# yixuan/spectra

Measured on AMD Instinct MI355X. Metric: eigenpairs_per_sec, higher is better.
Workload: dtype f64

## Files before the change

### include/mispec.h

```cpp
#ifndef MISPEC_H
#define MISPEC_H

#include <stdint.h>

#ifdef __cplusplus
extern "C" {
#endif

#define MISPEC_OK 0
#define MISPEC_EINVAL (-1)
#define MISPEC_ELOGIC (-2)
#define MISPEC_ERUNTIME (-3)

typedef struct mispec_ctx mispec_ctx;
typedef struct mispec_csr mispec_csr;
typedef struct mispec_fac mispec_fac;

const char* mispec_last_error(void);
const char* mispec_version(void);

int mispec_set_option(const char* name, const char* value);
const char* mispec_get_option(const char* name);

int mispec_ctx_create(int device, void* hip_stream, mispec_ctx** out);
// ... 25 lines not shown
int mispec_csr_from_csc(mispec_ctx* ctx, int64_t n_rows, int64_t n_cols, const int32_t* colptr_host,
                        const int32_t* rowind_host, const double* val_host, mispec_csr** out);
int mispec_csr_from_triangle(mispec_ctx* ctx, int64_t n, const int32_t* outer_host, const int32_t* inner_host,
                             const double* val_host, char uplo, int row_major, mispec_csr** out);
int mispec_csr_synth_band(mispec_ctx* ctx, int64_t n, uint64_t seed, const int64_t* offsets, int noff, int symmetric,
                          mispec_csr** out);
int mispec_csr_destroy(mispec_csr* A);
int64_t mispec_csr_rows(const mispec_csr* A);
int64_t mispec_csr_cols(const mispec_csr* A);
int64_t mispec_csr_local_rows(const mispec_csr* A);
int64_t mispec_csr_local_nnz(const mispec_csr* A);
int mispec_csr_offset_codes(const mispec_csr* A);
int mispec_csr_use_offset_codes(mispec_csr* A, int enable);
int mispec_csr_use_windows(mispec_csr* A, int enable);
int mispec_csr_windows_info(const mispec_csr* A, int64_t* blocks, int64_t* covered_entries, int64_t* lds_doubles);
int mispec_csr_windows_in_use(const mispec_csr* A);
int mispec_csr_windows_table(const mispec_csr* A, int32_t* records_out, int64_t capacity);
int mispec_csr_windows_host(int64_t n_rows, int64_t n_cols, int64_t row_begin, const int32_t* rowptr, const int32_t* colind,
                            int32_t* records_out);
int mispec_csr_spmv_format(const mispec_csr* A);
int mispec_csr_set_spmv_format(mispec_csr* A, int format);
double mispec_csr_spmv_bytes(const mispec_csr* A, int stored);
int mispec_csr_dia_info(const mispec_csr* A, int* ndia, int* nstored, int* nmirrored, int* lead_blocks);
int mispec_dia_sym_plan(const int32_t* offsets, int nd, int64_t reach, int32_t* out_flags, int* lead_blocks);
int mispec_csr_coeff(const mispec_csr* A, int64_t i, int64_t j, double* out);
int mispec_csr_download(const mispec_csr* A, int32_t* rowptr_host, int32_t* colind_host, double* val_host);

int mispec_spmv(const mispec_csr* A, const double* x_dev, double* y_dev);
int mispec_spmv_host(const mispec_csr* A, const double* x_host, double* y_host);
int mispec_spmm_host(const mispec_csr* A, const double* X_host, int64_t ldx, int k, double* Y_host, int64_t ldy);
int mispec_spmm(const mispec_csr* A, const double* X_dev, int64_t ldx, int k, double* Y_dev, int64_t ldy);
int mispec_spmm_plan(int k, int forced_panel, int* widths_out, int cap, int* count);
int mispec_csr_reorder(mispec_csr* A, int method, int* applied);
int mispec_csr_reordering(const mispec_csr* A, double* far_before, double* far_after);
int mispec_csr_permutation(const mispec_csr* A, int32_t* perm_out);
int mispec_csr_tiles_info(const mispec_csr* A, int64_t* segments, int64_t* entries, int64_t* padding, int64_t* chunks);
int mispec_csr_staged_info(const mispec_csr* A, int64_t* bins, int64_t* slots, int64_t* batches, int64_t* chunks);
int mispec_last_ingest_info(double* seconds_out, int count);
int mispec_ingest_threads(void);
int mispec_mirror_triangle_host(int64_t n, const int32_t* outer, const int32_t* inner, const double* val, char uplo, int row_major,
                                int32_t* rowptr_out, int32_t* colind_out, double* val_out, int64_t capacity, int64_t* nnz_out);
int mispec_tiles_spmv_host(int64_t nrows, int64_t ncols, const int32_t* rowptr, const int32_t* colind, const double* val,
                           const double* x, double* y, int* built, int64_t* stats);
int mispec_staged_spmv_host(int64_t nrows, int64_t ncols, const int32_t* rowptr, const int32_t* colind, const double* val,
                            const double* x, double* y, int* built, int64_t* stats);
int mispec_rcm_order(int64_t n, const int32_t* rowptr, const int32_t* colind, int symmetric_pattern, int32_t* perm_out,
// ... 177 lines not shown
```

### spectra_amd/__init__.py

```python
import ctypes as C
import enum
import os

import numpy as np

from . import _capi
from ._capi import MispecError, Profile, build_library, check, lib

__all__ = ["SortRule", "CompInfo", "Context", "SparseSymMatProd", "SparseGenMatProd", "SparseSymShiftSolve", "SymEigsSolver",
           "SymEigsShiftSolver", "GenEigsSolver", "SVDMatOp", "PartialSVDSolver", "SparseRegularInverse", "SparseCholesky", "SymGEigsSolver", "SymShiftInvert", "SymGEigsShiftSolver", "SparseGenRealShiftSolve", "GenEigsRealShiftSolver", "shard_block",
           "Factorization", "tridiag_qr", "tridiag_eigen", "hess_qr", "double_shift_qr", "hess_schur", "hess_eigen", "MispecError", "build_library", "shard_range", "BAND_OFFSETS", "SYNTH_SEED",
           "SparseHermMatProd", "DenseHermMatProd", "HermEigsSolver", "spmm_plan", "dia_sym_plan"]

BAND_OFFSETS = (1, 2, 3, 1000, 1001, 100000, 100001)
SYNTH_SEED = 20240607


ORTH_MODES = {"reference": 0, "onesweep": 1, "onesweep-eager": 1 | 0x100, "onesweep-recorrect": 1 | 0x200, "onesweep-restart-check": 1 | 0x400,
              "onesweep-onered": 1 | 0x800, "onesweep-twored": 1 | 0x1000, "onesweep-onered-eager": 1 | 0x800 | 0x100}


def _orth_mode_value(mode):
    if isinstance(mode, str):
        if mode not in ORTH_MODES:
# ... 252 lines not shown
        return ms.value

    def algorithmic_bytes(self):
        return 12.0 * self.nnz() + 4.0 * (self.local_rows() + 1) + 8.0 * self.cols() + 8.0 * self.local_rows()

    def offset_codes(self):
        return int(lib().mispec_csr_offset_codes(self.h))

    def use_offset_codes(self, enable=True):
        check(lib().mispec_csr_use_offset_codes(self.h, 1 if enable else 0))

    def use_windows(self, enable=True):
        check(lib().mispec_csr_use_windows(self.h, -1 if enable is None else (1 if enable else 0)))

    def windows_info(self):
        a, b, c = C.c_int64(0), C.c_int64(0), C.c_int64(0)
        check(lib().mispec_csr_windows_info(self.h, C.byref(a), C.byref(b), C.byref(c)))
        return {"blocks": a.value, "covered_entries": b.value, "lds_doubles": c.value}

    def dia_info(self):
        a, b, c, d = C.c_int(0), C.c_int(0), C.c_int(0), C.c_int(0)
        check(lib().mispec_csr_dia_info(self.h, C.byref(a), C.byref(b), C.byref(c), C.byref(d)))
        return {"ndia": a.value, "nstored": b.value, "nmirrored": c.value, "lead_blocks": d.value}

    def windows_in_use(self):
        return bool(lib().mispec_csr_windows_in_use(self.h))

    def windows_table(self):
        nb = (self.local_rows() + 255) // 256
        out = np.empty((nb, 32), dtype=np.int32)
        check(lib().mispec_csr_windows_table(self.h, _ip(out), out.size))
        return out

    def spmv_format(self):
        return int(lib().mispec_csr_spmv_format(self.h))

    def set_spmv_format(self, fmt=-1):
        check(lib().mispec_csr_set_spmv_format(self.h, int(fmt)))

    def stored_bytes(self):
        return float(lib().mispec_csr_spmv_bytes(self.h, 1))

    def staged_info(self):
        a, b, c, d = C.c_int64(0), C.c_int64(0), C.c_int64(0), C.c_int64(0)
        check(lib().mispec_csr_staged_info(self.h, C.byref(a), C.byref(b), C.byref(c), C.byref(d)))
        return {"bins": a.value, "slots": b.value, "batches": c.value, "chunks": d.value}
# ... 1393 lines not shown
```

### spectra_amd/_capi.py

```python
import ctypes as C
import os
import subprocess

_PKG = os.path.dirname(os.path.abspath(__file__))
LIB_PATH = os.path.join(_PKG, "libmispec.so")
EXTRAS_LIB_PATH = os.path.join(_PKG, "libmispec_extras.so")
EXTRAS_PREFIXES = ("mispec_davidson_", "mispec_zdense_", "mispec_zfac_", "mispec_zcsr_", "mispec_hermeigs_")
CSRC = os.path.join(_PKG, "csrc")

MISPEC_OK, MISPEC_EINVAL, MISPEC_ELOGIC, MISPEC_ERUNTIME = 0, -1, -2, -3


class MispecError(RuntimeError):
    """HIP / RCCL failure or a failed small decomposition (std::runtime_error in the C++ API)."""


def build_library(force=False, verbose=False):
    cmd = ["make", "-C", CSRC, "-j8"] + (["-B"] if force else [])
    out = subprocess.run(cmd, stdout=subprocess.PIPE, stderr=subprocess.STDOUT, text=True)
    if verbose or out.returncode != 0:
        print(out.stdout)
    if out.returncode != 0:
        raise RuntimeError("building libmispec.so failed")
    return LIB_PATH
# ... 44 lines not shown
    "mispec_loopback_destroy": (C.c_int, [_vp]),
    "mispec_shard_block": (C.c_int64, [C.c_int64, C.c_int]),
    "mispec_shard_range": (C.c_int, [C.c_int64, C.c_int, C.c_int, _lp, _lp]),
    "mispec_csr_upload": (C.c_int, [_vp, C.c_int64, C.c_int64, _ip, _ip, _dp, _vpp]),
    "mispec_csr_from_csc": (C.c_int, [_vp, C.c_int64, C.c_int64, _ip, _ip, _dp, _vpp]),
    "mispec_csr_from_triangle": (C.c_int, [_vp, C.c_int64, _ip, _ip, _dp, C.c_char, C.c_int, _vpp]),
    "mispec_csr_synth_band": (C.c_int, [_vp, C.c_int64, C.c_uint64, _lp, C.c_int, C.c_int, _vpp]),
    "mispec_csr_destroy": (C.c_int, [_vp]),
    "mispec_csr_rows": (C.c_int64, [_vp]),
    "mispec_csr_cols": (C.c_int64, [_vp]),
    "mispec_csr_local_rows": (C.c_int64, [_vp]),
    "mispec_csr_local_nnz": (C.c_int64, [_vp]),
    "mispec_csr_offset_codes": (C.c_int, [_vp]),
    "mispec_csr_use_offset_codes": (C.c_int, [_vp, C.c_int]),
    "mispec_csr_use_windows": (C.c_int, [_vp, C.c_int]),
    "mispec_csr_windows_info": (C.c_int, [_vp, _lp, _lp, _lp]),
    "mispec_csr_windows_table": (C.c_int, [_vp, _ip, C.c_int64]),
    "mispec_csr_windows_in_use": (C.c_int, [_vp]),
    "mispec_csr_windows_host": (C.c_int, [C.c_int64, C.c_int64, C.c_int64, _ip, _ip, _ip]),
    "mispec_csr_spmv_format": (C.c_int, [_vp]),
    "mispec_csr_set_spmv_format": (C.c_int, [_vp, C.c_int]),
    "mispec_csr_spmv_bytes": (C.c_double, [_vp, C.c_int]),
    "mispec_csr_dia_info": (C.c_int, [_vp, C.POINTER(C.c_int), C.POINTER(C.c_int), C.POINTER(C.c_int), C.POINTER(C.c_int)]),
    "mispec_dia_sym_plan": (C.c_int, [_ip, C.c_int, C.c_int64, _ip, C.POINTER(C.c_int)]),
    "mispec_csr_coeff": (C.c_int, [_vp, C.c_int64, C.c_int64, _dp]),
    "mispec_csr_download": (C.c_int, [_vp, _ip, _ip, _dp]),
    "mispec_spmv": (C.c_int, [_vp, _vp, _vp]),
    "mispec_spmv_host": (C.c_int, [_vp, _dp, _dp]),
    "mispec_spmm_host": (C.c_int, [_vp, _dp, C.c_int64, C.c_int, _dp, C.c_int64]),
    "mispec_spmv_time": (C.c_int, [_vp, _vp, _vp, C.c_int, C.POINTER(C.c_float)]),
    "mispec_spmm": (C.c_int, [_vp, _vp, C.c_int64, C.c_int, _vp, C.c_int64]),
    "mispec_spmm_time": (C.c_int, [_vp, _vp, C.c_int64, C.c_int, _vp, C.c_int64, C.c_int, C.POINTER(C.c_float)]),
    "mispec_spmm_plan": (C.c_int, [C.c_int, C.c_int, C.POINTER(C.c_int), C.c_int, C.POINTER(C.c_int)]),
    "mispec_symshift_level_plan": (C.c_int, [C.c_int64, C.c_int64, C.c_int, _lp, _lp, _lp, _lp]),
    "mispec_symshift_create": (C.c_int, [_vp, C.c_int64, _ip, _ip, _dp, C.c_char, C.c_int, _vpp]),
    "mispec_symshift_destroy": (C.c_int, [_vp]),
    "mispec_symshift_rows": (C.c_int64, [_vp]),
    "mispec_symshift_bandwidth": (C.c_int, [_vp, _lp, _lp, C.POINTER(C.c_int)]),
    "mispec_csr_tiles_info": (C.c_int, [_vp, _lp, _lp, _lp, _lp]),
    "mispec_csr_staged_info": (C.c_int, [_vp, _lp, _lp, _lp, _lp]),
    "mispec_csr_reorder": (C.c_int, [_vp, C.c_int, C.POINTER(C.c_int)]),
    "mispec_csr_reordering": (C.c_int, [_vp, _dp, _dp]),
    "mispec_csr_permutation": (C.c_int, [_vp, _ip]),
    "mispec_staged_spmv_host": (C.c_int, [C.c_int64, C.c_int64, _ip, _ip, _dp, _dp, _dp, C.POINTER(C.c_int), C.POINTER(C.c_int64)]),
    "mispec_tiles_spmv_host": (C.c_int, [C.c_int64, C.c_int64, _ip, _ip, _dp, _dp, _dp, C.POINTER(C.c_int), C.POINTER(C.c_int64)]),
    "mispec_rcm_order": (C.c_int, [C.c_int64, _ip, _ip, C.c_int, _ip, C.POINTER(C.c_int), C.POINTER(C.c_int64)]),
# ... 218 lines not shown
```

### spectra_amd/csrc/common.hpp

```cpp
#pragma once

#include <hip/hip_runtime.h>

#include <cstdint>
#include <cstdio>
#include <cstdlib>
#include <new>
#include <functional>
#include <utility>
#include <stdexcept>
#include <string>
#include <vector>

#include "../../include/mispec.h"
#include "../../include/mispec_extras.h"

namespace mispec {

struct Error : std::runtime_error
{
    int code;
    Error(int c, const std::string& m) : std::runtime_error(m), code(c) {}
};

// ... 88 lines not shown
    PinnedBuf() {}
    PinnedBuf(const PinnedBuf&) = delete;
    PinnedBuf& operator=(const PinnedBuf&) = delete;
    ~PinnedBuf()
    {
        if (p)
            (void) hipHostFree(p);
    }
    void alloc(size_t count)
    {
        if (p)
            (void) hipHostFree(p);
        p = nullptr;
        MISPEC_HIP(hipHostMalloc(reinterpret_cast<void**>(&p), count * sizeof(T), hipHostMallocDefault));
        n = count;
    }
};

inline int64_t round_up(int64_t x, int64_t m) { return (x + m - 1) / m * m; }

enum class Opt
{
    orth, one_reduction, orth_kernel, host_turn, small, restart_sync, host_steps, overlap, csr_win, spec_corr, exchange, reorder,
    spmv_staged, spmv_tiles, spmm, dia_sym, host_threads, shift, count
};
enum class Orth { onesweep, onesweep_eager, reference };
enum class OrthKernel { dma, dma2, reg, unset };
enum class HostTurn { fast, copy };
enum class Small { host, host_serial, device };
enum class Exchange { allgather, halo, unset };
enum class Reorder { automatic, rcm, none };
enum class Tri { automatic, off, on };
enum class DiaSym { automatic, off, all };
enum class Spmm { automatic, off, w2, w4, w8 };
int option_choice(Opt o);
template <typename E>
E option_choice(Opt o, E unset)
{
    const int i = option_choice(o);
    return i < 0 ? unset : E(i);
}
bool option_flag(Opt o, bool unset);
int option_int(Opt o, int unset);
struct ShiftOptions
{
    int lds = 1;
    int batch = 0;
    int lanes = 0;
    int block_inverse = 256;
    int factor_host = 0;
    int wave = 1;
    int profile = 0;
};
ShiftOptions shift_options();

void* big_host_alloc(size_t bytes);
// ... 57 lines not shown
```

### spectra_amd/csrc/csr_dia.hip

```cpp
#include "csr_kernels.hpp"

#include <algorithm>
#include <cstdlib>
#include <cstring>
#include <numeric>
#include <vector>

using namespace mispec;

namespace {

constexpr int kMaxDia = 32;
constexpr int kDiaGroup = 8;
constexpr int64_t kDiaSymReach = 131072;
constexpr bool kMirrorNontemporal = false;
constexpr int kDiaMir = 8;

__global__ __launch_bounds__(256) void k_build_dia(const int32_t* __restrict__ rowptr, const uint8_t* __restrict__ codes,
                                                   const double* __restrict__ val, const int32_t* __restrict__ pos_of_code,
                                                   int64_t nloc, int64_t ld, double* __restrict__ dia, int* __restrict__ bad, int nd_blocked)
{
    const int64_t r = int64_t(blockIdx.x) * 256 + threadIdx.x;
    if (r >= nloc)
        return;
// ... 490 lines not shown
        __syncthreads();
        const int wv = tid >> 6, lane = tid & 63;
#pragma unroll
        for (int h = 0; h < 2; h++)
        {
            const int k = 2 * wv + h;
            const double s = wave_reduce_sum(cbuf[64 * k + lane]);
            if (lane == 0)
                red[k] = s;
        }
        __syncthreads();
        if (tid == 0)
            epi.partials[lb] = (red[0] + red[1]) + (red[2] + red[3]);
    }
    else
    {
        if (have1)
            *reinterpret_cast<double2*>(y + row0 + r0) = make_double2(acc0, acc1);
        else if (have0)
            y[row0 + r0] = acc0;
    }
}

int dia_sym_rule(const int32_t* offs, int nd, int64_t reach, int32_t* flags)
{
    int64_t kmax = 0;
    for (int i = 0; i < nd; i++)
    {
        flags[i] = 0;
        const int64_t k = -int64_t(offs[i]);
        if (k <= 0 || (reach >= 0 && k > reach))
            continue;
        for (int j = 0; j < nd; j++)
            if (int64_t(offs[j]) == k)
                flags[i] = 1;
        if (flags[i])
            kmax = std::max(kmax, k);
    }
    return int((kmax + 255) / 256);
}

mispec_dia_plan make_plan(const int32_t* offs, int nd, const int32_t* mirrored)
{
    mispec_dia_plan pl;
    int64_t kmax = 0;
    for (int i = 0; i < nd; i++)
// ... 1 lines not shown
        pl.shift[i] = mirrored[i] ? -offs[i] : 0;
        if (!mirrored[i])
            pl.src[i] = pl.nstored++ + mispec_dia_plan::kStream;
        else
            kmax = std::max<int64_t>(kmax, -int64_t(offs[i]));
    }
    pl.lead = int((kmax + 255) / 256);
    for (int i = 0; i < nd; i++)
        if (mirrored[i])
            for (int j = 0; j < nd; j++)
                if (offs[j] == -offs[i])
                {
                    pl.src[j] = pl.slot(j);
                    pl.src[i] = pl.slot(j) + (kMirrorNontemporal ? mispec_dia_plan::kStream : 0);
                }
    for (int i = nd; i < 32; i++)
    {
        pl.src[i] = pl.src[nd - 1];
        pl.shift[i] = pl.shift[nd - 1];
    }
    return pl;
}

}

extern "C" int mispec_dia_sym_plan(const int32_t* offsets, int nd, int64_t reach, int32_t* out_flags, int* lead_blocks)
{
    return guarded([&] {
        MISPEC_REQUIRE(nd >= 0 && nd <= kMaxDia && (nd == 0 || (offsets && out_flags)), "mispec_dia_sym_plan: bad argument");
        const int lead = dia_sym_rule(offsets, nd, reach, out_flags);
        if (lead_blocks)
            *lead_blocks = lead;
    });
}

extern "C" int mispec_csr_dia_info(const mispec_csr* A, int* ndia, int* nstored, int* nmirrored, int* lead_blocks)
{
    return guarded([&] {
        MISPEC_REQUIRE(A, "mispec_csr_dia_info: NULL argument");
        if (ndia)
            *ndia = A->ndia;
        if (nstored)
            *nstored = A->ndia ? A->dia_plan.nstored : 0;
        if (nmirrored)
            *nmirrored = A->ndia ? A->ndia - A->dia_plan.nstored : 0;
        if (lead_blocks)
            *lead_blocks = A->ndia ? A->dia_plan.lead : 0;
    });
}

namespace mispec {

void build_dia(mispec_csr& A, const std::vector<int32_t>& dict)
{
    const int64_t nloc = A.local_rows();
    const int nd = int(dict.size());
    if (nd == 0 || nd > kMaxDia || nloc == 0 || double(A.nnz) < 0.75 * double(nd) * double(nloc))
        return;
    std::vector<int32_t> order(static_cast<size_t>(nd)), pos(static_cast<size_t>(nd)), offs(static_cast<size_t>(nd));
    std::iota(order.begin(), order.end(), 0);
    std::sort(order.begin(), order.end(), [&](int32_t a, int32_t b) { return dict[size_t(a)] < dict[size_t(b)]; });
    for (int k = 0; k < nd; k++)
    {
        pos[size_t(order[size_t(k)])] = k;
        offs[size_t(k)] = dict[size_t(order[size_t(k)])];
    }
    constexpr bool blocked = true;
    const int64_t ld = round_up(nloc, 256);
    DevBuf<int32_t> d_pos;
    DevBuf<int> d_bad;
// ... 87 lines not shown
    hipLaunchKernelGGL(k_dia_compact, dim3(nblk), dim3(256), 0, st, A.dia.p, nd, nloc, plan, packed.p);
    MISPEC_HIP(hipGetLastError());
    MISPEC_HIP(hipStreamSynchronize(st));
    A.dia.swap(packed);
    A.dia_plan = plan;
}

void launch_spmv_dia(const mispec_csr& A, const SpmvLaunch& L)
{
    const dim3 grid = L.grid, block = L.block;
    const int64_t nloc = L.nloc;
    const int nblocks = L.nblocks;
    const SpmvEpilogue* epi = L.epi;
    const SpmvEpilogue e = L.e;
    const hipEvent_t ev_start = L.ev_start, ev_stop = L.ev_stop;
    const double* x_dev = L.x_dev;
    double* y_dev = L.y_dev;
        const DiaArgs da{A.dia.p, A.dia_off.p, A.dia_ld, A.ndia, int(A.n_cols - 1), A.row_begin, A.dia_plan};
        const bool mir = A.dia_plan.nstored != A.ndia;
        MISPEC_REQUIRE(!mir || (A.dia_ld == 0 && A.dia_win.nc > 0), "diagonal storage: a mirror plan needs the block layout and x windows");
        const bool dia2 = A.dia_win.nc > 0 && A.dia_ld == 0 && A.ndia <= 2 * kDiaGroup &&
                          (reinterpret_cast<uintptr_t>(y_dev) & 15) == 0 &&
                          (!epi || ((reinterpret_cast<uintptr_t>(e.v_rows) & 15) == 0 && (reinterpret_cast<uintptr_t>(e.v_prev) & 15) == 0));
        if (dia2)
        {
            const size_t lds2 = size_t(A.dia_win.total + 256) * sizeof(double);
            const dim3 block2(128);
            const int ng = (A.ndia + kDiaGroup - 1) / kDiaGroup;
            const bool post = epi && e.post_scale_state;
#define MISPEC_DIA2_LAUNCH(E, G, W, P)                                                                                                  \
    do                                                                                                                                  \
    {                                                                                                                                   \
        if (ev_start && ev_stop)                                                                                                        \
            hipExtLaunchKernelGGL((k_spmv_dia_win2<E, G, W, P>), grid, block2, lds2, A.ctx->stream, ev_start, ev_stop, 0, da, A.dia_win, \
                                  x_dev, y_dev, nloc, nblocks, e);                                                                      \
        else                                                                                                                            \
            hipLaunchKernelGGL((k_spmv_dia_win2<E, G, W, P>), grid, block2, lds2, A.ctx->stream, da, A.dia_win, x_dev, y_dev, nloc,     \
                               nblocks, e);                                                                                             \
    } while (0)
#define MISPEC_DIA2_W(E, G, P)               \
    do                                       \
    {                                        \
        if (A.dia_win.nc <= 4)               \
            MISPEC_DIA2_LAUNCH(E, G, 4, P);  \
        else if (A.dia_win.nc <= 6)          \
            MISPEC_DIA2_LAUNCH(E, G, 6, P);  \
// ... 138 lines not shown
```

### spectra_amd/csrc/ctx.hip

```cpp
#include "common.hpp"

#include <dlfcn.h>
#include <rccl/rccl.h>

#include <algorithm>
#include <condition_variable>
#include <exception>
#include <thread>
#include <cstring>
#include <mutex>

namespace mispec {
static thread_local std::string g_last_error;
void set_last_error(const std::string& msg) { g_last_error = msg; }

void* big_host_alloc(size_t bytes)
{
    void* q = std::malloc(bytes ? bytes : 1);
    if (!q)
        throw std::bad_alloc();
    return q;
}

namespace {
// ... 18 lines not shown
    {Opt::orth_kernel, "orth_kernel", "MISPEC_ORTH_KERNEL", Kind::choice, {"dma", "dma2", "reg"}, 0, 0,
     "orthogonalisation passes through an LDS-DMA ring of three / two slots or through registers (unset: dma from 131072 rows)"},
    {Opt::host_turn, "host_turn", "MISPEC_HOST_TURN", Kind::choice, {"fast", "copy"}, 0, 0,
     "restart's host turn: pinned-memory kernels or hipMemcpy"},
    {Opt::small, "small", "MISPEC_SMALL", Kind::choice, {"host", "host-serial", "device"}, 0, 0,
     "where the ncv x ncv work of a restart runs"},
    {Opt::restart_sync, "restart_sync", "MISPEC_RESTART_SYNC", Kind::choice, {"0", "1"}, 0, 0, "synchronising fused restart"},
    {Opt::host_steps, "host_steps", "MISPEC_HOST_STEPS", Kind::choice, {"0", "1"}, 0, 0, "host-synchronous steps"},
    {Opt::overlap, "overlap", "MISPEC_OVERLAP", Kind::choice, {"0", "1"}, 0, 0,
     "sharded product: overlap of the exchange with the local rows (default 1)"},
    {Opt::csr_win, "csr_win", "MISPEC_CSR_WIN", Kind::choice, {"0", "1"}, 0, 0, "x windows of the int32 CSR kernel (default 1)"},
    {Opt::spec_corr, "spec_corr", "MISPEC_SPEC_CORR", Kind::integer, {}, 1, 4,
     "corrections enqueued speculatively per step (unset: 2, 1 when sharded)"},
    {Opt::exchange, "exchange", "MISPEC_EXCHANGE", Kind::choice, {"allgather", "halo"}, 0, 0,
     "sharded product: the all-gather or the neighbour exchange (unset: the exchange when the halos are small)"},
    {Opt::reorder, "reorder", "MISPEC_REORDER", Kind::choice, {"auto", "rcm", "none"}, 0, 0,
     "reverse Cuthill-McKee ordering at ingest and of the shift solve"},
    {Opt::spmv_staged, "spmv_staged", "MISPEC_SPMV_STAGED", Kind::choice, {"auto", "0", "1"}, 0, 0, "staged SpMV format"},
    {Opt::spmv_tiles, "spmv_tiles", "MISPEC_SPMV_TILES", Kind::choice, {"auto", "0", "1"}, 0, 0, "column-blocked tile SpMV format"},
    {Opt::spmm, "spmm", "MISPEC_SPMM", Kind::choice, {"auto", "0", "2", "4", "8"}, 0, 0,
     "widest panel of a block product (0: one SpMV per column)"},
    {Opt::dia_sym, "dia_sym", "MISPEC_DIA_SYM", Kind::choice, {"auto", "0", "all"}, 0, 0,
     "diagonal storage: lower diagonals read from their mirrored upper partner (auto: those within reach, 0: none, all)"},
    {Opt::host_threads, "host_threads", "MISPEC_HOST_THREADS", Kind::integer, {}, 1, kMaxInt,
     "upper bound on the host threads of the ingest and of the shift solve's host-side factorisation"},
    {Opt::shift, "shift", "MISPEC_SHIFT", Kind::shift, {}, 0, 0, "kernel variants of the banded shift solve"},
};
static_assert(sizeof(kOptions) / sizeof(kOptions[0]) == size_t(Opt::count), "one entry per option");
constexpr bool entries_in_order()
{
    for (size_t i = 0; i < size_t(Opt::count); i++)
        if (kOptions[i].id != Opt(i))
            return false;
    return true;
}
static_assert(entries_in_order(), "kOptions is indexed by Opt");

struct ShiftKey
{
    const char* key;
    const char* values[kMaxValues];
    int ShiftOptions::*field;
};
const ShiftKey kShiftKeys[] = {
    {"lds", {"0", "1"}, &ShiftOptions::lds},
    {"batch", {"8", "16", "32"}, &ShiftOptions::batch},
// ... 609 lines not shown
```

### spectra_amd/csrc/orth_dma.hip

```cpp
#include "krylov.hpp"

using namespace mispec;

namespace {

constexpr int kThreads = 256;
constexpr int kNW = 4;
constexpr int kRows = 128;
typedef __attribute__((address_space(3))) char lds_char;

__device__ __forceinline__ double wave_sum(double v)
{
#pragma unroll
    for (int off = 32; off > 0; off >>= 1)
        v += __shfl_down(v, off, 64);
    return v;
}
__device__ __forceinline__ double wave_max(double v)
{
#pragma unroll
    for (int off = 32; off > 0; off >>= 1)
        v = fmax(v, __shfl_down(v, off, 64));
    return v;
}

template <bool NT>
__device__ __forceinline__ void dma16(const double* gsrc, unsigned lds_dst)
{
    unsigned keep;
    if (NT)
        asm volatile("s_mov_b32 %0, m0\n\ts_mov_b32 m0, %2\n\ts_nop 0\n\tglobal_load_lds_dwordx4 %1, off nt\n\ts_mov_b32 m0, %0"
                     : "=&s"(keep)
                     : "v"(gsrc), "s"(lds_dst)
                     : "memory");
    else
        asm volatile("s_mov_b32 %0, m0\n\ts_mov_b32 m0, %2\n\ts_nop 0\n\tglobal_load_lds_dwordx4 %1, off\n\ts_mov_b32 m0, %0"
                     : "=&s"(keep)
                     : "v"(gsrc), "s"(lds_dst)
                     : "memory");
}

template <int MAXS, int DEPTH, bool ONERED>
__global__ __launch_bounds__(kThreads, 1) void k_orth_lagged_dma(OrthArgs a)
{
    constexpr int NL = MAXS + 1;
    constexpr int kRegion = kRows;
    constexpr int kSlotDoubles = kNW * NL * kRegion;
    extern __shared__ __attribute__((aligned(16))) char smem[];
    double* ring = reinterpret_cast<double*>(smem);
    double* psum = ring + DEPTH * kSlotDoubles;
    double* cs = psum + 2 * kNW * kRows;

    if (a.status && *a.status != kStepOk)
        return;
    const int tid = threadIdx.x;
    const int lane = tid & 63;
    const int w = __builtin_amdgcn_readfirstlane(tid >> 6);
    const bool pending = *a.pending != 0;
    const double alpha = *a.alpha_dev;
    const double beta = *a.beta_dev;
    if (tid < 64)
        cs[tid] = (pending && tid < a.ncol) ? a.c_in[tid] : 0.0;
// ... 231 lines not shown
```

### spectra_amd/csrc/orth_dma_modes.hip

```cpp
#include "krylov.hpp"

using namespace mispec;

namespace {

constexpr int kThreads = 256;
constexpr int kNW = 4;
constexpr int kRows = 128;
typedef __attribute__((address_space(3))) char lds_char;

__device__ __forceinline__ double wave_sum(double v)
{
#pragma unroll
    for (int off = 32; off > 0; off >>= 1)
        v += __shfl_down(v, off, 64);
    return v;
}
__device__ __forceinline__ double wave_max(double v)
{
#pragma unroll
    for (int off = 32; off > 0; off >>= 1)
        v = fmax(v, __shfl_down(v, off, 64));
    return v;
}

template <bool NT>
__device__ __forceinline__ void dma16(const double* gsrc, unsigned lds_dst)
{
    unsigned keep;
    if (NT)
        asm volatile("s_mov_b32 %0, m0\n\ts_mov_b32 m0, %2\n\ts_nop 0\n\tglobal_load_lds_dwordx4 %1, off nt\n\ts_mov_b32 m0, %0"
                     : "=&s"(keep)
                     : "v"(gsrc), "s"(lds_dst)
                     : "memory");
    else
        asm volatile("s_mov_b32 %0, m0\n\ts_mov_b32 m0, %2\n\ts_nop 0\n\tglobal_load_lds_dwordx4 %1, off\n\ts_mov_b32 m0, %0"
                     : "=&s"(keep)
                     : "v"(gsrc), "s"(lds_dst)
                     : "memory");
}

template <int MODE, int MAXS, int DEPTH>
__global__ __launch_bounds__(kThreads, 1) void k_orth_dma(OrthArgs a)
{
    constexpr bool kCorrect = (MODE == ORTH_CORRECT_VTF || MODE == ORTH_CORRECT_ONLY);
    constexpr bool kVtf = (MODE != ORTH_CORRECT_ONLY);
    constexpr int NL = MAXS + 1;
    constexpr int kRegion = kRows;
    constexpr int kSlotDoubles = kNW * NL * kRegion;
    extern __shared__ __attribute__((aligned(16))) char smem[];
    double* ring = reinterpret_cast<double*>(smem);
    double* psum = ring + DEPTH * kSlotDoubles;
    double* cs = psum + 2 * kNW * kRows;

    if (a.status && *a.status != kStepOk)
        return;
    if (a.need_corr && *a.need_corr == 0)
        return;
    const int tid = threadIdx.x;
    const int lane = tid & 63;
    const int w = __builtin_amdgcn_readfirstlane(tid >> 6);
    double alpha = 0.0;
// ... 225 lines not shown
```

Measured before the change: 22.22.

## Add persistent streamed DIA SpMV kernel with LDS DMA ring pipelining

Adds a persistent DIA SpMV kernel for matrices whose lower diagonals are mirrored from upper ones. Each workgroup takes a strided set of row blocks, with blocks grouped per XCD. Diagonal, x-window and vector tiles are prefetched into a multi-slot LDS ring with global_load_lds DMA, so memory traffic overlaps the compute of earlier blocks. It is chosen automatically for large local row counts or through a new dia_kernel option, and the shared DMA helper moves to a header. The cost is complex indexing, edge handling and a heavy LDS footprint of one workgroup per CU.

```diff
diff --git a/include/mispec.h b/include/mispec.h
--- a/include/mispec.h
+++ b/include/mispec.h
@@ -71,6 +71,7 @@
 int mispec_csr_set_spmv_format(mispec_csr* A, int format);
 double mispec_csr_spmv_bytes(const mispec_csr* A, int stored);
 int mispec_csr_dia_info(const mispec_csr* A, int* ndia, int* nstored, int* nmirrored, int* lead_blocks);
+int mispec_csr_dia_kernel_info(const mispec_csr* A, int* kernel, int* grid);
 int mispec_dia_sym_plan(const int32_t* offsets, int nd, int64_t reach, int32_t* out_flags, int* lead_blocks);
 int mispec_csr_coeff(const mispec_csr* A, int64_t i, int64_t j, double* out);
 int mispec_csr_download(const mispec_csr* A, int32_t* rowptr_host, int32_t* colind_host, double* val_host);
diff --git a/spectra_amd/__init__.py b/spectra_amd/__init__.py
--- a/spectra_amd/__init__.py
+++ b/spectra_amd/__init__.py
@@ -298,6 +298,11 @@
         a, b, c, d = C.c_int(0), C.c_int(0), C.c_int(0), C.c_int(0)
         check(lib().mispec_csr_dia_info(self.h, C.byref(a), C.byref(b), C.byref(c), C.byref(d)))
         return {"ndia": a.value, "nstored": b.value, "nmirrored": c.value, "lead_blocks": d.value}
+
+    def dia_kernel_info(self):
+        k, g = C.c_int(0), C.c_int(0)
+        check(lib().mispec_csr_dia_kernel_info(self.h, C.byref(k), C.byref(g)))
+        return {"kernel": "stream" if k.value else "block", "stream_grid": g.value}
 
     def windows_in_use(self):
         return bool(lib().mispec_csr_windows_in_use(self.h))
diff --git a/spectra_amd/_capi.py b/spectra_amd/_capi.py
--- a/spectra_amd/_capi.py
+++ b/spectra_amd/_capi.py
@@ -90,6 +90,7 @@
     "mispec_csr_set_spmv_format": (C.c_int, [_vp, C.c_int]),
     "mispec_csr_spmv_bytes": (C.c_double, [_vp, C.c_int]),
     "mispec_csr_dia_info": (C.c_int, [_vp, C.POINTER(C.c_int), C.POINTER(C.c_int), C.POINTER(C.c_int), C.POINTER(C.c_int)]),
+    "mispec_csr_dia_kernel_info": (C.c_int, [_vp, C.POINTER(C.c_int), C.POINTER(C.c_int)]),
     "mispec_dia_sym_plan": (C.c_int, [_ip, C.c_int, C.c_int64, _ip, C.POINTER(C.c_int)]),
     "mispec_csr_coeff": (C.c_int, [_vp, C.c_int64, C.c_int64, _dp]),
     "mispec_csr_download": (C.c_int, [_vp, _ip, _ip, _dp]),
diff --git a/spectra_amd/csrc/common.hpp b/spectra_amd/csrc/common.hpp
--- a/spectra_amd/csrc/common.hpp
+++ b/spectra_amd/csrc/common.hpp
@@ -134,7 +134,7 @@
 enum class Opt
 {
     orth, one_reduction, orth_kernel, host_turn, small, restart_sync, host_steps, overlap, csr_win, spec_corr, exchange, reorder,
-    spmv_staged, spmv_tiles, spmm, dia_sym, host_threads, shift, count
+    spmv_staged, spmv_tiles, spmm, dia_sym, dia_kernel, host_threads, shift, count
 };
 enum class Orth { onesweep, onesweep_eager, reference };
 enum class OrthKernel { dma, dma2, reg, unset };
@@ -144,6 +144,7 @@
 enum class Reorder { automatic, rcm, none };
 enum class Tri { automatic, off, on };
 enum class DiaSym { automatic, off, all };
+enum class DiaKernel { automatic, block, stream };
 enum class Spmm { automatic, off, w2, w4, w8 };
 int option_choice(Opt o);
 template <typename E>
diff --git a/spectra_amd/csrc/csr_dia.hip b/spectra_amd/csrc/csr_dia.hip
--- a/spectra_amd/csrc/csr_dia.hip
+++ b/spectra_amd/csrc/csr_dia.hip
@@ -1,4 +1,5 @@
 #include "csr_kernels.hpp"
+#include "lds_dma.hpp"
 
 #include <algorithm>
 #include <cstdlib>
@@ -536,6 +537,286 @@
     }
 }
 
+constexpr int kStreamThreads = 256;
+constexpr int kStreamMaxInstr = 16;
+constexpr int kStreamLds = 160 * 1024 - 1024;
+constexpr int kStreamDepthMax = 3;
+
+struct DiaStream
+{
+    int ni = 0;
+    int first_x = 0, first_vprev = -1, first_vrows = -1, first_tail = 0;
+    int ntail = 0;
+    int depth = 0;
+    int off_lo = 0, off_hi = 0;
+    int xpar[8];
+    int xtail[8], xcnt[8];
+    int xc[2 * kDiaGroup];
+    int xrel[2 * kDiaGroup];
+    int mtail[2 * kDiaGroup];
+};
+
+__host__ __device__ inline void dia_stream_blocks(int wg, int G, int nblocks, int& first, int& count)
+{
+    const int per = (nblocks + 7) >> 3, Gx = G >> 3;
+    const int xcd = wg & 7, j = wg >> 3;
+    const int rest = nblocks - xcd * per, have = rest < per ? rest : per;
+    first = xcd * per + j;
+    count = j < have ? (have - j + Gx - 1) / Gx : 0;
+}
+
+__device__ __forceinline__ void dia_stream_wait(int keep)
+{
+    switch (keep)
+    {
+#define MISPEC_WAIT_CASE(N) \
+    case N:                 \
+        asm volatile("s_waitcnt vmcnt(" #N ")" ::: "memory"); \
+        break;
+        MISPEC_WAIT_CASE(1) MISPEC_WAIT_CASE(2) MISPEC_WAIT_CASE(3) MISPEC_WAIT_CASE(4) MISPEC_WAIT_CASE(5) MISPEC_WAIT_CASE(6)
+        MISPEC_WAIT_CASE(7) MISPEC_WAIT_CASE(8) MISPEC_WAIT_CASE(9) MISPEC_WAIT_CASE(10) MISPEC_WAIT_CASE(11) MISPEC_WAIT_CASE(12)
+        MISPEC_WAIT_CASE(13) MISPEC_WAIT_CASE(14) MISPEC_WAIT_CASE(15) MISPEC_WAIT_CASE(16)
+#undef MISPEC_WAIT_CASE
+        default:
+            asm volatile("s_waitcnt vmcnt(0)" ::: "memory");
+    }
+}
+
+template <bool EPI, int NG, int NCW = 8, bool POST = false>
+__global__ __launch_bounds__(kStreamThreads, 1) void k_spmv_dia_stream(DiaArgs da, mispec_dia_windows w, DiaStream sp,
+                                                                       const double* __restrict__ x, double* __restrict__ y,
+                                                                       int64_t nrows, int nblocks, SpmvEpilogue epi)
+{
+    extern __shared__ __attribute__((aligned(16))) char smem[];
+    __shared__ double red[2][4];
+    constexpr int NV = (NG % kDiaMir) * kDiaGroup;
+    static_assert(NV <= 2 * kDiaGroup, "the streamed kernel keeps at most sixteen diagonals");
+    if (EPI && epi.status && *epi.status != 0)
+        return;
+    const int tid = threadIdx.x, lane = tid & 63;
+    const int wv = __builtin_amdgcn_readfirstlane(tid >> 6);
+    double beta = 1.0;
+    if (POST)
+    {
+        StepState* st = static_cast<StepState*>(epi.post_scale_state);
+        beta = st->beta;
+        const bool first = (blockIdx.x == 0 && tid == 0);
+        if (beta < epi.post_scale_eps_sqrt)
+        {
+            if (first)
+            {
+                st->status = kStepSmallBeta;
+                st->stop_step = epi.post_scale_step;
+                st->stop_count = 0;
+            }
+            return;
+        }
+        if (first)
+            st->subd[epi.post_scale_step - 1] = beta;
+    }
+    int lm0, nmine;
+    dia_stream_blocks(int(blockIdx.x), int(gridDim.x), nblocks, lm0, nmine);
+    if (nmine <= 0)
+        return;
+    const int Gx = int(gridDim.x) >> 3;
+    const int lb0 = epi.first_block + lm0;
+    const int nd = da.nd, nc = w.nc;
+    const int col_max = da.col_max;
+    const bool have_vprev = EPI && epi.v_prev != nullptr;
+
+    double x_lo = x[0], x_hi = x[col_max], hprev = 0.0;
+    if (have_vprev)
+        hprev = POST ? beta : (epi.h_prev_dev ? *epi.h_prev_dev : epi.h_prev);
+
+    const int tail0 = sp.first_tail * 128;
+    int voff[NV], xoff[NV], coff[NV];
+#pragma unroll
+    for (int k = 0; k < NV; k++)
+    {
+        const int kk = min(k, nd - 1);
+        const int q = tid + (da.plan.shift[kk] & 1);
+        voff[k] = q < 256 ? kk * 256 + q : tail0 + 2 * sp.mtail[kk];
+        const int c = sp.xc[kk];
+        const int i = sp.xrel[kk] + sp.xpar[c] + tid;
+        xoff[k] = i < 256 ? (sp.first_x + 2 * c) * 128 + i : tail0 + 2 * sp.xtail[c] + (i - 256);
+        coff[k] = w.start[c] + sp.xrel[kk] + tid;
+    }
+
+    const int nwi = __builtin_amdgcn_readfirstlane((sp.ni - wv + 3) >> 2);
+    const double* ibase[kStreamMaxInstr];
+    int64_t icur[kStreamMaxInstr], istep[kStreamMaxInstr], ilo[kStreamMaxInstr], ihi[kStreamMaxInstr];
+    unsigned iflags = 0;
+    {
+        const int64_t xa = int64_t(reinterpret_cast<uintptr_t>(x) >> 3) & 1;
+        const int64_t xlo = xa;
+        int64_t xhi = int64_t(col_max) - 1;
+        if ((xhi + xa) & 1)
+            xhi--;
+        const int64_t vhi = 2 * ((nrows >> 1) - 1);
+        const int64_t mstep = int64_t(Gx) * da.plan.nstored * 256, vstep = int64_t(Gx) * 256;
+        const int64_t e0 = (int64_t(da.plan.lead) + lb0) * 256;
+        const int64_t r0 = int64_t(lb0) * 256;
+        const auto mat = [&](int k, int j) {
+            const int shift = da.plan.shift[k];
+            const int64_t e = e0 + 2 * j - shift - (shift & 1);
+            return ((e >> 8) * da.plan.nstored + da.plan.slot(k)) * 256 + (e & 255);
+        };
+        const auto xel = [&](int c, int j) { return da.row_begin + r0 + w.start[c] - sp.xpar[c] + 2 * j; };
+#pragma unroll
+        for (int jj = 0; jj < kStreamMaxInstr; jj++)
+        {
+            const int i = wv + 4 * jj;
+            ibase[jj] = x;
+            icur[jj] = xlo;
+            istep[jj] = 0;
+            ilo[jj] = xlo;
+            ihi[jj] = xhi;
+            if (i >= sp.ni)
+                continue;
+            if (i < sp.first_x)
+            {
+                const int k = i >> 1;
+                ibase[jj] = da.dia;
+                icur[jj] = mat(k, 64 * (i & 1) + lane);
+                istep[jj] = mstep;
+                if (da.plan.src[k] & mispec_dia_plan::kStream)
+                    iflags |= 1u << jj;
+            }
+            else if (i < sp.first_x + 2 * nc)
+            {
+                const int c = (i - sp.first_x) >> 1;
+                icur[jj] = xel(c, 64 * ((i - sp.first_x) & 1) + lane);
+                istep[jj] = vstep;
+                iflags |= 0x10000u << jj;
+            }
+            else if (i < sp.first_tail)
+            {
+                const bool prev = sp.first_vprev >= 0 && i < sp.first_vprev + 2;
+                const int h = i - (prev ? sp.first_vprev : sp.first_vrows);
+                ibase[jj] = prev ? epi.v_prev : epi.v_rows;
+                icur[jj] = r0 + 2 * (64 * h + lane);
+                istep[jj] = vstep;
+                ilo[jj] = 0;
+                ihi[jj] = vhi;
+                iflags |= 0x10000u << jj;
+            }
+            else
+            {
+                const int t = 64 * (i - sp.first_tail) + lane;
+                iflags |= 0x10000u << jj;
+                for (int k = 0; k < nd; k++)
+                    if (sp.mtail[k] == t)
+                    {
+                        ibase[jj] = da.dia;
+                        icur[jj] = mat(k, 128);
+                        istep[jj] = mstep;
+                        ilo[jj] = 0;
+                        ihi[jj] = int64_t(0x7fffffffffffffff);
+                    }
+                for (int c = 0; c < nc; c++)
+                    if (t >= sp.xtail[c] && t < sp.xtail[c] + sp.xcnt[c])
+                    {
+                        icur[jj] = xel(c, 128 + t - sp.xtail[c]);
+                        istep[jj] = vstep;
+                    }
+            }
+        }
+    }
+    asm volatile("s_waitcnt vmcnt(0) lgkmcnt(0)" : "+v"(x_lo), "+v"(x_hi), "+v"(hprev), "+v"(beta)::"memory");
+
+    const unsigned lds0 = static_cast<unsigned>(reinterpret_cast<uintptr_t>((lds_char*) smem));
+    const unsigned slot_bytes = unsigned(sp.ni) * 1024u;
+    const double* ring = reinterpret_cast<const double*>(smem);
+    const int depth = sp.depth;
+
+    const auto issue = [&](int slot) {
+        const unsigned sbase = __builtin_amdgcn_readfirstlane(lds0 + unsigned(slot) * slot_bytes + unsigned(wv) * 1024u);
+#pragma unroll
+        for (int jj = 0; jj < kStreamMaxInstr; jj++)
+            if (jj < nwi)
+            {
+                int64_t idx = icur[jj];
+                icur[jj] += istep[jj];
+                if (iflags & (0x10000u << jj))
+                    idx = min(max(idx, ilo[jj]), ihi[jj]);
+                if (iflags & (1u << jj))
+                    dma16<true>(ibase[jj] + idx, sbase + unsigned(jj) * 4096u);
+                else
+                    dma16<false>(ibase[jj] + idx, sbase + unsigned(jj) * 4096u);
+            }
+    };
+
+    for (int p = 0; p < depth - 1 && p < nmine; p++)
+        issue(p);
+    int slot = 0;
+    for (int it = 0; it < nmine; it++)
+    {
+        const int ahead = min(depth - 2, nmine - 1 - it);
+        dia_stream_wait(nwi * ahead);
+        asm volatile("s_waitcnt lgkmcnt(0)\n\ts_barrier" ::: "memory");
+        if (it + depth - 1 < nmine)
+            issue(slot == 0 ? depth - 1 : slot - 1);
+        const int lb = lb0 + it * Gx;
+        if (EPI && it > 0 && tid == 0)
+            epi.partials[lb - Gx] = (red[(it - 1) & 1][0] + red[(it - 1) & 1][1]) + (red[(it - 1) & 1][2] + red[(it - 1) & 1][3]);
+        const int64_t row0 = int64_t(lb) * 256;
+        const int nr = int(min(int64_t(256), nrows - row0));
+        const int64_t g0 = da.row_begin + row0;
+        const double* S = ring + size_t(slot) * (slot_bytes / 8);
+        const bool edge = g0 + sp.off_lo <= 1 || g0 + 255 + sp.off_hi >= int64_t(col_max) - 1;
+        double acc = 0.0;
+        if (edge)
+        {
+#pragma unroll
+            for (int k = 0; k < NV; k++)
+                if (k < nd)
+                {
+                    const int64_t col = g0 + coff[k];
+                    double xv = S[xoff[k]];
+                    xv = col <= 0 ? x_lo : (col >= col_max ? x_hi : xv);
+                    acc = add_rounded_product(acc, S[voff[k]], xv);
+                }
+        }
+        else
+        {
+#pragma unroll
+            for (int k = 0; k < NV; k++)
+                if (k < nd)
+                    acc = add_rounded_product(acc, S[voff[k]], S[xoff[k]]);
+        }
+        if (EPI)
+        {
+            double contrib = 0.0;
+            if (tid < nr)
+            {
+                const int64_t row = row0 + tid;
+                const bool direct = nr < 256;
+                double yv = POST ? acc / beta : acc;
+                if (have_vprev)
+                    yv -= hprev * (direct ? epi.v_prev[row] : S[sp.first_vprev * 128 + tid]);
+                y[row] = yv;
+                double vr = direct ? epi.v_rows[row] : S[sp.first_vrows * 128 + tid];
+                if (POST)
+                    vr = vr / beta;
+                contrib = vr * yv;
+            }
+            const double s = wave_reduce_sum(contrib);
+            if (lane == 0)
+                red[it & 1][wv] = s;
+        }
+        else if (tid < nr)
+            y[row0 + tid] = acc;
+        slot = slot + 1 == depth ? 0 : slot + 1;
+    }
+    if (EPI)
+    {
+        __syncthreads();
+        if (tid == 0)
+            epi.partials[lb0 + (nmine - 1) * Gx] =
+                (red[(nmine - 1) & 1][0] + red[(nmine - 1) & 1][1]) + (red[(nmine - 1) & 1][2] + red[(nmine - 1) & 1][3]);
+    }
+}
+
 int dia_sym_rule(const int32_t* offs, int nd, int64_t reach, int32_t* flags)
 {
     int64_t kmax = 0;
@@ -583,6 +864,78 @@
     return pl;
 }
 
+
+constexpr int64_t kStreamMinRows = int64_t(1) << 20;
+
+bool make_dia_stream(const mispec_csr& A, const double* x_dev, bool epi, bool vprev, DiaStream& sp)
+{
+    const mispec_dia_windows& w = A.dia_win;
+    const mispec_dia_plan& pl = A.dia_plan;
+    const int nd = A.ndia;
+    if (nd < 1 || nd > 2 * kDiaGroup || w.nc < 1 || A.dia_ld != 0 || A.n_cols < 4 || A.local_rows() < 2)
+        return false;
+    sp = DiaStream();
+    sp.first_x = 2 * nd;
+    int i = 2 * nd + 2 * w.nc;
+    if (epi)
+    {
+        if (vprev)
+        {
+            sp.first_vprev = i;
+            i += 2;
+        }
+        sp.first_vrows = i;
+        i += 2;
+    }
+    sp.first_tail = i;
+    int t = 0;
+    for (int k = 0; k < 2 * kDiaGroup; k++)
+        sp.mtail[k] = (k < nd && (pl.shift[k] & 1)) ? t++ : -1;
+    const int64_t xa = int64_t(reinterpret_cast<uintptr_t>(x_dev) >> 3) & 1;
+    for (int c = 0; c < 8; c++)
+    {
+        sp.xpar[c] = sp.xtail[c] = sp.xcnt[c] = 0;
+        if (c >= w.nc)
+            continue;
+        sp.xpar[c] = int((xa + A.row_begin + w.start[c]) & 1);
+        sp.xtail[c] = t;
+        sp.xcnt[c] = (sp.xpar[c] + w.len[c] + 1) / 2 - 128;
+        t += sp.xcnt[c];
+    }
+    for (int k = 0; k < 2 * kDiaGroup; k++)
+    {
+        const int kk = std::min(k, nd - 1);
+        int c = 0;
+        while (c + 1 < w.nc && w.base[c + 1] <= w.idx[kk])
+            c++;
+        sp.xc[k] = c;
+        sp.xrel[k] = w.idx[kk] - w.base[c];
+    }
+    sp.off_lo = w.start[0];
+    sp.off_hi = w.start[w.nc - 1] + w.len[w.nc - 1] - 256;
+    sp.ntail = t;
+    sp.ni = sp.first_tail + (t + 63) / 64;
+    if ((sp.ni + 3) / 4 > kStreamMaxInstr)
+        return false;
+    sp.depth = kStreamDepthMax;
+    while (sp.depth >= 2 && sp.depth * sp.ni * 1024 > kStreamLds)
+        sp.depth--;
+    return sp.depth >= 2;
+}
+
+int dia_stream_grid(const mispec_csr& A, int nblocks)
+{
+    const int per = (nblocks + 7) >> 3;
+    return 8 * std::max(1, std::min(A.ctx->num_cu / 8, per));
+}
+
+bool dia_stream_wanted(const mispec_csr& A)
+{
+    const DiaKernel dk = option_choice(Opt::dia_kernel, DiaKernel::automatic);
+    if (dk == DiaKernel::block || A.ndia == 0 || A.dia_plan.nstored == A.ndia)
+        return false;
+    return dk == DiaKernel::stream || A.local_rows() >= kStreamMinRows;
+}
 }
 
 extern "C" int mispec_dia_sym_plan(const int32_t* offsets, int nd, int64_t reach, int32_t* out_flags, int* lead_blocks)
@@ -607,6 +960,20 @@
             *nmirrored = A->ndia ? A->ndia - A->dia_plan.nstored : 0;
         if (lead_blocks)
             *lead_blocks = A->ndia ? A->dia_plan.lead : 0;
+    });
+}
+
+extern "C" int mispec_csr_dia_kernel_info(const mispec_csr* A, int* kernel, int* grid)
+{
+    return guarded([&] {
+        MISPEC_REQUIRE(A, "mispec_csr_dia_kernel_info: NULL argument");
+        DiaStream sp;
+        const bool win2 = A->ndia && A->dia_win.nc > 0 && A->dia_ld == 0 && A->ndia <= 2 * kDiaGroup;
+        const bool stream = win2 && dia_stream_wanted(*A) && make_dia_stream(*A, nullptr, true, true, sp);
+        if (kernel)
+            *kernel = stream ? 1 : 0;
+        if (grid)
+            *grid = stream ? dia_stream_grid(*A, spmv_num_blocks(A->local_rows())) : 0;
     });
 }
 
@@ -740,6 +1107,60 @@
         const bool dia2 = A.dia_win.nc > 0 && A.dia_ld == 0 && A.ndia <= 2 * kDiaGroup &&
                           (reinterpret_cast<uintptr_t>(y_dev) & 15) == 0 &&
                           (!epi || ((reinterpret_cast<uintptr_t>(e.v_rows) & 15) == 0 && (reinterpret_cast<uintptr_t>(e.v_prev) & 15) == 0));
+        DiaStream sp;
+        if (dia2 && mir && nblocks >= 1 && dia_stream_wanted(A) && make_dia_stream(A, x_dev, epi != nullptr, epi && e.v_prev, sp))
+        {
+            const size_t ldss = size_t(sp.depth) * size_t(sp.ni) * 1024;
+            const dim3 grids(unsigned(dia_stream_grid(A, nblocks))), blocks(kStreamThreads);
+            const int ng = (A.ndia + kDiaGroup - 1) / kDiaGroup;
+            const bool post = epi && e.post_scale_state;
+#define MISPEC_DIAS_LAUNCH(E, G, W, P)                                                                                                   \
+    do                                                                                                                                  \
+    {                                                                                                                                   \
+        static thread_local int attr_dev = -1;                                        \
+        if (attr_dev != A.ctx->device)                                                                                                  \
+        {                                                                                                                               \
+            MISPEC_HIP(hipFuncSetAttribute(reinterpret_cast<const void*>(&k_spmv_dia_stream<E, G, W, P>),                               \
+                                           hipFuncAttributeMaxDynamicSharedMemorySize, kStreamLds));                                   \
+            attr_dev = A.ctx->device;                                                                                                   \
+        }                                                                                                                               \
+        if (ev_start && ev_stop)                                                                                                        \
+            hipExtLaunchKernelGGL((k_spmv_dia_stream<E, G, W, P>), grids, blocks, ldss, A.ctx->stream, ev_start, ev_stop, 0, da,        \
+                                  A.dia_win, sp, x_dev, y_dev, nloc, nblocks, e);                                                       \
+        else                                                                                                                            \
+            hipLaunchKernelGGL((k_spmv_dia_stream<E, G, W, P>), grids, blocks, ldss, A.ctx->stream, da, A.dia_win, sp, x_dev, y_dev,    \
+                               nloc, nblocks, e);                                                                                       \
+    } while (0)
+#define MISPEC_DIAS_W(E, G, P)               \
+    do                                       \
+    {                                        \
+        if (A.dia_win.nc <= 4)               \
+            MISPEC_DIAS_LAUNCH(E, G, 4, P);  \
+        else if (A.dia_win.nc <= 6)          \
+            MISPEC_DIAS_LAUNCH(E, G, 6, P);  \
+        else                                 \
+            MISPEC_DIAS_LAUNCH(E, G, 8, P);  \
+    } while (0)
+#define MISPEC_DIAS_G(E, P)                    \
+    do                                         \
+    {                                          \
+        if (ng == 1)                           \
+            MISPEC_DIAS_W(E, kDiaMir + 1, P);  \
+        else                                   \
+            MISPEC_DIAS_W(E, kDiaMir + 2, P);  \
+    } while (0)
+            if (post)
+                MISPEC_DIAS_G(true, true);
+            else if (epi)
+                MISPEC_DIAS_G(true, false);
+            else
+                MISPEC_DIAS_G(false, false);
+#undef MISPEC_DIAS_G
+#undef MISPEC_DIAS_W
+#undef MISPEC_DIAS_LAUNCH
+            MISPEC_HIP(hipGetLastError());
+            return;
+        }
         if (dia2)
         {
             const size_t lds2 = size_t(A.dia_win.total + 256) * sizeof(double);
diff --git a/spectra_amd/csrc/ctx.hip b/spectra_amd/csrc/ctx.hip
--- a/spectra_amd/csrc/ctx.hip
+++ b/spectra_amd/csrc/ctx.hip
@@ -64,6 +64,8 @@
      "widest panel of a block product (0: one SpMV per column)"},
     {Opt::dia_sym, "dia_sym", "MISPEC_DIA_SYM", Kind::choice, {"auto", "0", "all"}, 0, 0,
      "diagonal storage: lower diagonals read from their mirrored upper partner (auto: those within reach, 0: none, all)"},
+    {Opt::dia_kernel, "dia_kernel", "MISPEC_DIA_KERNEL", Kind::choice, {"auto", "block", "stream"}, 0, 0,
+     "diagonal storage with mirrored diagonals: one workgroup per row block or the persistent, streamed kernel (auto: by size)"},
     {Opt::host_threads, "host_threads", "MISPEC_HOST_THREADS", Kind::integer, {}, 1, kMaxInt,
      "upper bound on the host threads of the ingest and of the shift solve's host-side factorisation"},
     {Opt::shift, "shift", "MISPEC_SHIFT", Kind::shift, {}, 0, 0, "kernel variants of the banded shift solve"},
diff --git a/spectra_amd/csrc/lds_dma.hpp b/spectra_amd/csrc/lds_dma.hpp
--- /dev/null
+++ b/spectra_amd/csrc/lds_dma.hpp
@@ -0,0 +1,24 @@
+#pragma once
+#include <hip/hip_runtime.h>
+
+namespace {
+
+typedef __attribute__((address_space(3))) char lds_char;
+
+template <bool NT>
+__device__ __forceinline__ void dma16(const double* gsrc, unsigned lds_dst)
+{
+    unsigned keep;
+    if (NT)
+        asm volatile("s_mov_b32 %0, m0\n\ts_mov_b32 m0, %2\n\ts_nop 0\n\tglobal_load_lds_dwordx4 %1, off nt\n\ts_mov_b32 m0, %0"
+                     : "=&s"(keep)
+                     : "v"(gsrc), "s"(lds_dst)
+                     : "memory");
+    else
+        asm volatile("s_mov_b32 %0, m0\n\ts_mov_b32 m0, %2\n\ts_nop 0\n\tglobal_load_lds_dwordx4 %1, off\n\ts_mov_b32 m0, %0"
+                     : "=&s"(keep)
+                     : "v"(gsrc), "s"(lds_dst)
+                     : "memory");
+}
+
+}
diff --git a/spectra_amd/csrc/orth_dma.hip b/spectra_amd/csrc/orth_dma.hip
--- a/spectra_amd/csrc/orth_dma.hip
+++ b/spectra_amd/csrc/orth_dma.hip
@@ -1,4 +1,5 @@
 #include "krylov.hpp"
+#include "lds_dma.hpp"
 
 using namespace mispec;
 
@@ -7,7 +8,6 @@
 constexpr int kThreads = 256;
 constexpr int kNW = 4;
 constexpr int kRows = 128;
-typedef __attribute__((address_space(3))) char lds_char;
 
 __device__ __forceinline__ double wave_sum(double v)
 {
@@ -22,22 +22,6 @@
     for (int off = 32; off > 0; off >>= 1)
         v = fmax(v, __shfl_down(v, off, 64));
     return v;
-}
-
-template <bool NT>
-__device__ __forceinline__ void dma16(const double* gsrc, unsigned lds_dst)
-{
-    unsigned keep;
-    if (NT)
-        asm volatile("s_mov_b32 %0, m0\n\ts_mov_b32 m0, %2\n\ts_nop 0\n\tglobal_load_lds_dwordx4 %1, off nt\n\ts_mov_b32 m0, %0"
-                     : "=&s"(keep)
-                     : "v"(gsrc), "s"(lds_dst)
-                     : "memory");
-    else
-        asm volatile("s_mov_b32 %0, m0\n\ts_mov_b32 m0, %2\n\ts_nop 0\n\tglobal_load_lds_dwordx4 %1, off\n\ts_mov_b32 m0, %0"
-                     : "=&s"(keep)
-                     : "v"(gsrc), "s"(lds_dst)
-                     : "memory");
 }
 
 template <int MAXS, int DEPTH, bool ONERED>
diff --git a/spectra_amd/csrc/orth_dma_modes.hip b/spectra_amd/csrc/orth_dma_modes.hip
--- a/spectra_amd/csrc/orth_dma_modes.hip
+++ b/spectra_amd/csrc/orth_dma_modes.hip
@@ -1,4 +1,5 @@
 #include "krylov.hpp"
+#include "lds_dma.hpp"
 
 using namespace mispec;
 
@@ -7,7 +8,6 @@
 constexpr int kThreads = 256;
 constexpr int kNW = 4;
 constexpr int kRows = 128;
-typedef __attribute__((address_space(3))) char lds_char;
 
 __device__ __forceinline__ double wave_sum(double v)
 {
@@ -22,22 +22,6 @@
     for (int off = 32; off > 0; off >>= 1)
         v = fmax(v, __shfl_down(v, off, 64));
     return v;
-}
-
-template <bool NT>
-__device__ __forceinline__ void dma16(const double* gsrc, unsigned lds_dst)
-{
-    unsigned keep;
-    if (NT)
-        asm volatile("s_mov_b32 %0, m0\n\ts_mov_b32 m0, %2\n\ts_nop 0\n\tglobal_load_lds_dwordx4 %1, off nt\n\ts_mov_b32 m0, %0"
-                     : "=&s"(keep)
-                     : "v"(gsrc), "s"(lds_dst)
-                     : "memory");
-    else
-        asm volatile("s_mov_b32 %0, m0\n\ts_mov_b32 m0, %2\n\ts_nop 0\n\tglobal_load_lds_dwordx4 %1, off\n\ts_mov_b32 m0, %0"
-                     : "=&s"(keep)
-                     : "v"(gsrc), "s"(lds_dst)
-                     : "memory");
 }
 
 template <int MODE, int MAXS, int DEPTH>
```

New measurement: 16.66. 25.0% lower.
